# QualityMinds/cistgcn

Measured on AMD Instinct MI355X. Metric: sequences/sec (fwd+bwd) H3.6M 22-joint 50->25, higher is better.
Workload: dtype f32; 1 GPU; cistgcn64_b256_t50_v22; C=64, per_gpu_batch=256, global_batch=256, T_in=50, T_out=25, V=22, parallelism=dp1, graph=True, graph_branches=True, capture_kept=median, mixed_batches=False

## Files before the change

cistgcn_amd/_lib.py:

```python
import ctypes
import os
from ctypes import POINTER, c_double, c_float, c_int, c_int32, c_longlong, c_uint, c_ulonglong, c_void_p

HERE = os.path.dirname(os.path.abspath(__file__))
LIB_PATH = os.path.join(HERE, "libcistgcn_hip.so")

_handle = None
STAT_REPLICAS = 16
ALPHA_SLOTS = 64
_host_pointers_ok = False


class View4(ctypes.Structure):
    _fields_ = [("n", c_longlong * 4), ("s", c_longlong * 4)]


class NormAct(ctypes.Structure):
    _fields_ = [
        ("x", c_void_p), ("xv", View4),
        ("y", c_void_p), ("yv", View4),
        ("pre", c_void_p),
        ("add", c_void_p), ("av", View4),
        ("add_post", c_int),
        ("bn_mode", c_int),
# ... 209 lines not shown
    "cg_gate_head_scratch_floats": [c_int, c_int, c_int],
    "cg_context_heads_fwd": [POINTER(CtxHeads), P],
    "cg_context_heads_bwd": [POINTER(CtxHeads), P],
    "cg_context_heads_red_doubles": [c_int],
    "cg_map2adj_tail_fwd": [POINTER(AdjTail), c_int, c_int, P],
    "cg_map2adj_tail_bwd": [POINTER(AdjTail), c_int, c_int, P],
    "cg_map2adj_tail_ws_floats": [c_int],
    "cg_map2adj_tail_part_floats": [c_int, c_int, c_int],
    "cg_map2adj_tail_red_doubles": [c_int],
    "cg_augment_sequences": [P, P, P, P, P, P, P, P, P, P, c_int, c_int, c_int, c_int, P],
    "cg_map2adj_tail_geometry": [c_int, c_int, c_int, POINTER(c_int)],
    "cg_dstd_tail_geometry": [c_int, c_int, c_int, c_int, POINTER(c_int)],
    "cg_pointwise_maps_geometry": [c_int, c_int, c_int, c_int, POINTER(c_int), c_int, POINTER(c_int)],
    "cg_collapse_geometry": [c_int, c_int, c_int, c_int, c_int, c_int, POINTER(c_int)],
    "cg_fpn_conv_geometry": [c_int, c_int, c_int, c_int, c_int, POINTER(c_int)],
    "cg_stgcn_domain_geometry": [c_int, c_int, c_int, c_int, c_int, c_int, c_int, c_int, POINTER(c_int)],
    "cg_block_input_geometry": [c_int, c_int, c_int, c_int, POINTER(c_int)],
    "cg_norm_act_rows_per_block": [POINTER(View4)],
    "cg_glue_geometry": [c_int, c_int, c_int, POINTER(c_int)],
    "cg_mpjpe_sample_fwd": [P, P, P, c_int, c_int, P],
    "cg_mpjpe_sample_bwd": [P, P, P, P, c_int, c_int, P],
    "cg_attack_step": [POINTER(AttackStep), P],
    "cg_attack_step_max_floats": [],
    "cg_eval_metrics": [POINTER(EvalMetricsArgs), P],
    "cg_eval_metrics_ws_doubles": [c_int, c_int, c_int],
    "cg_attack_metrics": [POINTER(AttackMetricsArgs), P],
    "cg_attack_metrics_ws_doubles": [c_int, c_int, c_int],
    "cg_adam_flat": [P, P, P, P, LL, c_float, c_float, c_float, c_float, c_float, c_float, c_float, LL, P],
}
EXPORTS = tuple(sorted(_SIGNATURES))
# ... 33 lines not shown
```

cistgcn_amd/csrc/fpn_conv.hip:

```cpp
#include "cg_common.h"
#include "cg_phase.h"
#include "fpn_conv.h"

HIP_DYNAMIC_SHARED(unsigned char, cg_dyn_lds)

__device__ __forceinline__ void cg_fpn_store_quad(float* row, int p, int P, float a, float b, float c, float d) {
  if (p >= P) return;
  if ((P & 3) == 0) { *reinterpret_cast<float4*>(row + p) = make_float4(a, b, c, d); return; }
  *reinterpret_cast<float2*>(row + p) = make_float2(a, b);
  if (p + 2 < P) *reinterpret_cast<float2*>(row + p + 2) = make_float2(c, d);
}

#define CG_FPN_THREADS 512
#define CG_FPN_PAD 3

struct CgFpnGeom {
  int HP, WP, IMG;
  int P, PM;
  int K, KP, KS;
  int K2, KP2, KS2;
  int OM, CM;
  int per;
};
struct CgFpnArgs { CgFpnConv t; CgFpnGeom g; };

template <typename L, typename S>
__device__ __forceinline__ void cg_fpn_stage(int n, L load, S store) {
  for (int e0 = threadIdx.x; e0 < n; e0 += 8 * CG_FPN_THREADS) {
    float v[8];
#pragma unroll
    for (int j = 0; j < 8; ++j) { const int e = e0 + CG_FPN_THREADS * j; v[j] = e < n ? load(e) : 0.f; }
#pragma unroll
    for (int j = 0; j < 8; ++j) { const int e = e0 + CG_FPN_THREADS * j; if (e < n) store(e, v[j]); }
  }
}

__device__ __forceinline__ void cg_fpn_zero(float* img, int floats) {
  for (int e = threadIdx.x; e < floats / 4; e += CG_FPN_THREADS) reinterpret_cast<float4*>(img)[e] = make_float4(0.f, 0.f, 0.f, 0.f);
}
__device__ __forceinline__ void cg_fpn_fill(const float* __restrict__ src, long long sc, long long sh, int n, int H, int W, const CgFpnGeom& g, float* img) {
  const int P = H * W;
  cg_fpn_stage(n * P,
               [&](int e) { const int c = e / P, p = e - c * P, h = p / W; return src[c * sc + h * sh + (p - h * W)]; },
               [&](int e, float v) { const int c = e / P, p = e - c * P, h = p / W; img[c * g.IMG + (h + CG_FPN_PAD) * g.WP + (p - h * W) + CG_FPN_PAD] = v; });
}
__device__ __forceinline__ int cg_fpn_posoff(int p, int W, const CgFpnGeom& g) { const int h = p / W; return (h + CG_FPN_PAD) * g.WP + (p - h * W) + CG_FPN_PAD; }

__global__ __launch_bounds__(CG_FPN_THREADS) void cg_fpn_fwd_kernel(CgFpnArgs a) {
  const CgFpnConv& t = a.t; const CgFpnGeom& g = a.g;
  const int b = blockIdx.x, di = blockIdx.y, d = t.dil[di];
  float* sX = reinterpret_cast<float*>(cg_dyn_lds);
  float* sW = sX + t.C * g.IMG;
  int* sTap = reinterpret_cast<int*>(sW + g.OM * g.KS);
  int* sPos = sTap + g.KP;
  const int tid = threadIdx.x, lane = tid & 63, wave = __builtin_amdgcn_readfirstlane(tid >> 6), l15 = lane & 15, slot = lane >> 4;
  cg_fpn_zero(sX, t.C * g.IMG);
  cg_fpn_zero(sW, g.OM * g.KS);
  __syncthreads();
  cg_fpn_fill(t.x + (long long)b * t.xs[0], t.xs[1], t.xs[2], t.C, t.H, t.W, g, sX);
  cg_fpn_stage(t.O * g.K, [&](int e) { return t.w[di][e]; }, [&](int e, float v) { const int o = e / g.K; sW[o * g.KS + e - o * g.K] = v; });
  for (int k = tid; k < g.KP; k += CG_FPN_THREADS) {
    const int c = k / 9, ij = k - 9 * c, i = ij / 3, j = ij - 3 * i;
    sTap[k] = k < g.K ? c * g.IMG + d * (i - 1) * g.WP + d * (j - 1) : 0;
  }
  for (int p = tid; p < g.PM; p += CG_FPN_THREADS) sPos[p] = cg_fpn_posoff(p < g.P ? p : 0, t.W, g);
  __syncthreads();
  const int PT = g.PM / 16, OT = g.OM / 16, pairs = (PT + 1) / 2;
  float* yb = t.y[di] + (long long)b * t.O * g.P;
  for (int w = wave; w < pairs * OT; w += CG_FPN_THREADS / 64) {
    const int pr = w / OT, ot = w - pr * OT, pt0 = 2 * pr, pt1 = min(PT - 1, pt0 + 1);
    const int pa = sPos[16 * pt0 + l15], pb = sPos[16 * pt1 + l15];
    cg_f32x4 c0 = cg_f32x4{0.f, 0.f, 0.f, 0.f}, c1 = c0;
    const float* wp = sW + (16 * ot + l15) * g.KS + 4 * slot;
    for (int k0 = 0; k0 < g.KP; k0 += 16) {
      const float4 w4 = *reinterpret_cast<const float4*>(wp + k0);
      const int4 t4 = *reinterpret_cast<const int4*>(sTap + k0 + 4 * slot);
      const float wv[4] = {w4.x, w4.y, w4.z, w4.w};
      const int tv[4] = {t4.x, t4.y, t4.z, t4.w};
#pragma unroll
      for (int s = 0; s < 4; ++s) {
        c0 = __builtin_amdgcn_mfma_f32_16x16x4f32(sX[pa + tv[s]], wv[s], c0, 0, 0, 0);
        c1 = __builtin_amdgcn_mfma_f32_16x16x4f32(sX[pb + tv[s]], wv[s], c1, 0, 0, 0);
      }
    }
    const int o = 16 * ot + l15;
    if (o < t.O) {
      const float bias = t.bias[di] ? t.bias[di][o] : 0.f;
#pragma unroll
      for (int h = 0; h < 2; ++h) {
        if (h == 1 && pt1 == pt0) break;
        const int p = 16 * (h ? pt1 : pt0) + 4 * slot;
        const cg_f32x4 c = h ? c1 : c0;
        cg_fpn_store_quad(yb + (long long)o * g.P, p, g.P, c[0] + bias, c[1] + bias, c[2] + bias, c[3] + bias);
      }
    }
  }
}

#define CG_FPN_DXT 14

__global__ __launch_bounds__(CG_FPN_THREADS) void cg_fpn_dx_kernel(CgFpnArgs a) {
  const CgFpnConv& t = a.t; const CgFpnGeom& g = a.g;
  const int b = blockIdx.x;
  float* sD = reinterpret_cast<float*>(cg_dyn_lds);
  float* sW = sD + t.O * g.IMG;
  int* sTap = reinterpret_cast<int*>(sW + g.CM * g.KS2);
  int* sPos = sTap + g.KP2;
  const int tid = threadIdx.x, lane = tid & 63, wave = __builtin_amdgcn_readfirstlane(tid >> 6), l15 = lane & 15, slot = lane >> 4, nw = CG_FPN_THREADS / 64;
  const int PT = g.PM / 16, CT = g.CM / 16;
  cg_f32x4 acc[CG_FPN_DXT];
#pragma unroll
  for (int u = 0; u < CG_FPN_DXT; ++u) acc[u] = cg_f32x4{0.f, 0.f, 0.f, 0.f};
  for (int p = tid; p < g.PM; p += CG_FPN_THREADS) sPos[p] = cg_fpn_posoff(p < g.P ? p : 0, t.W, g);
  cg_fpn_zero(sD, t.O * g.IMG);
  cg_fpn_zero(sW, g.CM * g.KS2);
  for (int di = 0; di < t.n; ++di) {
    const int d = t.dil[di];
    __syncthreads();
    cg_fpn_fill(t.dy[di] + (long long)b * t.O * g.P, g.P, t.W, t.O, t.H, t.W, g, sD);
    cg_fpn_stage(t.O * t.C * 9, [&](int e) { return t.w[di][e]; },
                 [&](int e, float v) { const int oc = e / 9, ij = e - 9 * oc, o = oc / t.C, c = oc - o * t.C; sW[c * g.KS2 + o * 9 + ij] = v; });
    for (int k = tid; k < g.KP2; k += CG_FPN_THREADS) {
      const int o = k / 9, ij = k - 9 * o, i = ij / 3, j = ij - 3 * i;
      sTap[k] = k < g.K2 ? o * g.IMG - d * (i - 1) * g.WP - d * (j - 1) : 0;
    }
    __syncthreads();
#pragma unroll
    for (int u = 0; u < CG_FPN_DXT; u += 2) {
      const int id0 = u * nw + wave, id1 = (u + 1) * nw + wave;
      if (id0 < PT * CT) {
        const bool two = id1 < PT * CT;
        const int pt0 = id0 / CT, ct0 = id0 - pt0 * CT, pt1 = two ? id1 / CT : pt0, ct1 = two ? id1 - pt1 * CT : ct0;
        const int pa = sPos[16 * pt0 + l15], pb = sPos[16 * pt1 + l15];
        const float* wp0 = sW + (16 * ct0 + l15) * g.KS2 + 4 * slot;
        const float* wp1 = sW + (16 * ct1 + l15) * g.KS2 + 4 * slot;
        cg_f32x4 c0 = acc[u], c1 = acc[u + 1];
#pragma unroll 3
        for (int k0 = 0; k0 < g.KP2; k0 += 16) {
          const float4 w0 = *reinterpret_cast<const float4*>(wp0 + k0), w1 = *reinterpret_cast<const float4*>(wp1 + k0);
          const int4 t4 = *reinterpret_cast<const int4*>(sTap + k0 + 4 * slot);
          const float a0[4] = {sD[pa + t4.x], sD[pa + t4.y], sD[pa + t4.z], sD[pa + t4.w]};
          const float a1[4] = {sD[pb + t4.x], sD[pb + t4.y], sD[pb + t4.z], sD[pb + t4.w]};
          const float v0[4] = {w0.x, w0.y, w0.z, w0.w}, v1[4] = {w1.x, w1.y, w1.z, w1.w};
#pragma unroll
          for (int s4 = 0; s4 < 4; ++s4) {
            c0 = __builtin_amdgcn_mfma_f32_16x16x4f32(a0[s4], v0[s4], c0, 0, 0, 0);
            c1 = __builtin_amdgcn_mfma_f32_16x16x4f32(a1[s4], v1[s4], c1, 0, 0, 0);
          }
        }
        acc[u] = c0;
        if (two) acc[u + 1] = c1;
      }
    }
  }
  float* dxb = t.dx + (long long)b * t.C * g.P;
#pragma unroll
  for (int u = 0; u < CG_FPN_DXT; ++u) {
    const int id = u * nw + wave;
    if (id < PT * CT) {
      const int pt = id / CT, ct = id - pt * CT, c = 16 * ct + l15, p = 16 * pt + 4 * slot;
      if (c < t.C) cg_fpn_store_quad(dxb + (long long)c * g.P, p, g.P, acc[u][0], acc[u][1], acc[u][2], acc[u][3]);
    }
  }
}

#define CG_FPN_DWT 16

__global__ __launch_bounds__(CG_FPN_THREADS) void cg_fpn_dw_kernel(CgFpnArgs a) {
  const CgFpnConv& t = a.t; const CgFpnGeom& g = a.g;
  const int di = blockIdx.y, d = t.dil[di];
  const int b0 = blockIdx.x * g.per, b1 = min(t.B, b0 + g.per);
  if (b0 >= t.B) return;
  const int DS = g.PM + 4;
  float* sX = reinterpret_cast<float*>(cg_dyn_lds);
  float* sD = sX + t.C * g.IMG;
  int* sTap = reinterpret_cast<int*>(sD + g.OM * DS);
  int* sPos = sTap + g.KP;
  const int tid = threadIdx.x, lane = tid & 63, wave = __builtin_amdgcn_readfirstlane(tid >> 6), l15 = lane & 15, slot = lane >> 4, nw = CG_FPN_THREADS / 64;
  const int OT = g.OM / 16, KT = g.KP / 16;
  cg_f32x4 acc[CG_FPN_DWT];
#pragma unroll
  for (int u = 0; u < CG_FPN_DWT; ++u) acc[u] = cg_f32x4{0.f, 0.f, 0.f, 0.f};
  float bsum = 0.f, bsum1 = 0.f;
  for (int k = tid; k < g.KP; k += CG_FPN_THREADS) {
    const int c = k / 9, ij = k - 9 * c, i = ij / 3, j = ij - 3 * i;
    sTap[k] = k < g.K ? c * g.IMG + d * (i - 1) * g.WP + d * (j - 1) : 0;
  }
  for (int p = tid; p < g.PM; p += CG_FPN_THREADS) sPos[p] = cg_fpn_posoff(p < g.P ? p : 0, t.W, g);
  for (int e = tid; e < g.OM * DS; e += CG_FPN_THREADS) sD[e] = 0.f;
  cg_fpn_zero(sX, t.C * g.IMG);
  for (int b = b0; b < b1; ++b) {
    __syncthreads();
    cg_fpn_fill(t.x + (long long)b * t.xs[0], t.xs[1], t.xs[2], t.C, t.H, t.W, g, sX);
    const float* dyb = t.dy[di] + (long long)b * t.O * g.P;
    if ((g.P & 3) == 0) {
#pragma unroll 4
      for (int e = tid; e < t.O * (g.P / 4); e += CG_FPN_THREADS) {
        const int o = e / (g.P / 4), p = 4 * (e - o * (g.P / 4));
        *reinterpret_cast<float4*>(sD + o * DS + p) = *reinterpret_cast<const float4*>(dyb + (long long)o * g.P + p);
      }
    } else {
#pragma unroll 4
      for (int e = tid; e < t.O * (g.P / 2); e += CG_FPN_THREADS) {
        const int o = e / (g.P / 2), p = 2 * (e - o * (g.P / 2));
        *reinterpret_cast<float2*>(sD + o * DS + p) = *reinterpret_cast<const float2*>(dyb + (long long)o * g.P + p);
      }
    }
    __syncthreads();
#pragma unroll
    for (int u = 0; u < CG_FPN_DWT; u += 2) {
      const int id0 = u * nw + wave, id1 = (u + 1) * nw + wave;
      if (id0 < OT * KT) {
        const bool two = id1 < OT * KT;
        const int ot0 = id0 / KT, kt0 = id0 - ot0 * KT, ot1 = two ? id1 / KT : ot0, kt1 = two ? id1 - ot1 * KT : kt0;
        const int tap0 = sTap[16 * kt0 + l15], tap1 = sTap[16 * kt1 + l15];
        const float* dp0 = sD + (16 * ot0 + l15) * DS + 4 * slot;
        const float* dp1 = sD + (16 * ot1 + l15) * DS + 4 * slot;
        cg_f32x4 c0 = acc[u], c1 = acc[u + 1];
        float bs0 = 0.f, bs1 = 0.f;
#pragma unroll 2
        for (int p0 = 0; p0 < g.PM; p0 += 16) {
          const float4 d0 = *reinterpret_cast<const float4*>(dp0 + p0), d1 = *reinterpret_cast<const float4*>(dp1 + p0);
          const int4 q4 = *reinterpret_cast<const int4*>(sPos + p0 + 4 * slot);
          const float x0[4] = {sX[tap0 + q4.x], sX[tap0 + q4.y], sX[tap0 + q4.z], sX[tap0 + q4.w]};
          const float x1[4] = {sX[tap1 + q4.x], sX[tap1 + q4.y], sX[tap1 + q4.z], sX[tap1 + q4.w]};
          const float e0[4] = {d0.x, d0.y, d0.z, d0.w}, e1[4] = {d1.x, d1.y, d1.z, d1.w};
          bs0 += (d0.x + d0.y) + (d0.z + d0.w); bs1 += (d1.x + d1.y) + (d1.z + d1.w);
#pragma unroll
          for (int s4 = 0; s4 < 4; ++s4) {
            c0 = __builtin_amdgcn_mfma_f32_16x16x4f32(e0[s4], x0[s4], c0, 0, 0, 0);
            c1 = __builtin_amdgcn_mfma_f32_16x16x4f32(e1[s4], x1[s4], c1, 0, 0, 0);
          }
        }
        acc[u] = c0;
        if (two) acc[u + 1] = c1;
        if (kt0 == 0) { if (ot0) bsum1 += bs0; else bsum += bs0; }
        if (two && kt1 == 0) { if (ot1) bsum1 += bs1; else bsum += bs1; }
      }
    }
  }
  float* ws = t.ws + ((long long)blockIdx.x * t.n + di) * (t.O * g.K + t.O);
#pragma unroll
  for (int u = 0; u < CG_FPN_DWT; ++u) {
    const int id = u * nw + wave;
    if (id < OT * KT) {
      const int ot = id / KT, kt = id - ot * KT, k = 16 * kt + l15;
#pragma unroll
      for (int q = 0; q < 4; ++q) {
        const int o = 16 * ot + 4 * slot + q;
        if (o < t.O && k < g.K) ws[o * g.K + k] = acc[u][q];
      }
    }
  }
  bsum += __shfl_xor(bsum, 16, 64); bsum += __shfl_xor(bsum, 32, 64);
  bsum1 += __shfl_xor(bsum1, 16, 64); bsum1 += __shfl_xor(bsum1, 32, 64);
  float* sB = reinterpret_cast<float*>(cg_dyn_lds);
  __syncthreads();
  if (slot == 0) { sB[wave * 16 + l15] = bsum; sB[(nw + wave) * 16 + l15] = bsum1; }
  __syncthreads();
  if (tid < 32 && tid < t.O) {
    float s0 = 0.f;
// ... 6 lines not shown
  __shared__ float red[4][64];
  const CgFpnConv& t = a.t; const CgFpnGeom& g = a.g;
  const int di = blockIdx.y, n = t.O * g.K + t.O, e = blockIdx.x * 64 + (threadIdx.x & 63), part = threadIdx.x >> 6;
  float s = 0.f;
  if (e < n)
    for (int w = part; w < nwg; w += 4) s += t.ws[((long long)w * t.n + di) * n + e];
  red[part][threadIdx.x & 63] = s;
  __syncthreads();
  if (part == 0 && e < n) {
    s = (red[0][threadIdx.x] + red[1][threadIdx.x]) + (red[2][threadIdx.x] + red[3][threadIdx.x]);
    if (e < t.O * g.K) { if (t.dw[di]) t.dw[di][e] = s; }
    else if (t.db[di]) t.db[di][e - t.O * g.K] = s;
  }
}

static int cg_fpn_geometry(const CgFpnConv* t, CgFpnGeom* g) {
  if (!t || t->n <= 0 || t->n > 3) return CG_EARG;
  if (t->B <= 0 || t->C <= 0 || t->C > 64 || t->O <= 0 || t->O > 32 || t->H <= 0 || t->W <= 0) return CG_ESHAPE;
  for (int i = 0; i < t->n; ++i) if (t->dil[i] < 1 || t->dil[i] > CG_FPN_PAD) return CG_ESHAPE;
  g->HP = t->H + 2 * CG_FPN_PAD; g->WP = t->W + 2 * CG_FPN_PAD; g->IMG = g->HP * g->WP;
  g->P = t->H * t->W; g->PM = (g->P + 15) & ~15;
  if ((g->P & 1) || g->PM > 256) return CG_ESHAPE;
  g->K = t->C * 9; g->KP = (g->K + 15) & ~15; g->KS = g->KP + 4;
  g->K2 = t->O * 9; g->KP2 = (g->K2 + 15) & ~15; g->KS2 = g->KP2 + 4;
  g->OM = (t->O + 15) & ~15; g->CM = (t->C + 15) & ~15;
  const int nwg = t->B < 170 ? t->B : 170;
  g->per = (t->B + nwg - 1) / nwg;
  if ((g->PM / 16) * (g->CM / 16) > CG_FPN_DXT * 4) return CG_ESHAPE;
  if ((g->OM / 16) * (g->KP / 16) > CG_FPN_DWT * 4) return CG_ESHAPE;
  return CG_OK;
}
static size_t cg_fpn_lds_fwd(const CgFpnConv* t, const CgFpnGeom& g) { return ((size_t)t->C * g.IMG + (size_t)g.OM * g.KS + g.KP + g.PM) * 4; }
static size_t cg_fpn_lds_dx(const CgFpnConv* t, const CgFpnGeom& g) { return ((size_t)t->O * g.IMG + (size_t)g.CM * g.KS2 + g.KP2 + g.PM) * 4; }
static size_t cg_fpn_lds_dw(const CgFpnConv* t, const CgFpnGeom& g) { return ((size_t)t->C * g.IMG + (size_t)g.OM * (g.PM + 4) + g.KP + g.PM) * 4; }

static int cg_fpn_dw_nwg(int B, const CgFpnGeom& g) { return (B + g.per - 1) / g.per; }
extern "C" int cg_fpn_conv_geometry(int B, int C, int O, int H, int W, int* out) {
  if (!out) return CG_EARG;
  CgFpnConv t = {};
  t.B = B; t.C = C; t.O = O; t.H = H; t.W = W; t.n = 1; t.dil[0] = 1;
  CgFpnGeom g;
  const int st = cg_fpn_geometry(&t, &g);
  if (st != CG_OK) return st;
  out[0] = g.per; out[1] = cg_fpn_dw_nwg(B, g);
  return CG_OK;
}

extern "C" int cg_fpn_conv_supported(int B, int C, int O, int H, int W) {
  CgFpnConv t = {};
  t.B = B; t.C = C; t.O = O; t.H = H; t.W = W; t.n = 1; t.dil[0] = 1;
  CgFpnGeom g;
  if (cg_fpn_geometry(&t, &g) != CG_OK) return 0;
  const size_t cap = 160 * 1024;
  return cg_fpn_lds_fwd(&t, g) <= cap && cg_fpn_lds_dx(&t, g) <= cap && cg_fpn_lds_dw(&t, g) <= cap;
}
extern "C" long long cg_fpn_conv_ws_floats(int B, int C, int O, int n) { return (long long)(B < 170 ? B : 170) * n * (O * C * 9 + O); }

extern "C" int cg_fpn_conv_fwd(const CgFpnConv* t, void* stream_) {
  CgFpnArgs a;
  int st = cg_fpn_geometry(t, &a.g);
  if (st != CG_OK) return st;
  a.t = *t;
  if (!t->x) return CG_EARG;
  for (int i = 0; i < t->n; ++i) if (!t->w[i] || !t->y[i]) return CG_EARG;
  const size_t lds = cg_fpn_lds_fwd(t, a.g);
  if (lds > 160 * 1024) return CG_ESHAPE;
  hipError_t e = cg_lds_limit((const void*)cg_fpn_fwd_kernel, lds);
  if (e != hipSuccess) return (int)e;
  hipLaunchKernelGGL(cg_fpn_fwd_kernel, dim3((unsigned)t->B, (unsigned)t->n), dim3(CG_FPN_THREADS), lds, (hipStream_t)stream_, a);
  return cg_launch_status();
}

extern "C" int cg_fpn_conv_bwd(const CgFpnConv* t, void* stream_) {
  CgFpnArgs a;
  int st = cg_fpn_geometry(t, &a.g);
  if (st != CG_OK) return st;
  a.t = *t;
  if (!t->x || !t->ws) return CG_EARG;
  for (int i = 0; i < t->n; ++i) if (!t->w[i] || !t->dy[i]) return CG_EARG;
  hipStream_t stream = (hipStream_t)stream_;
  if (t->dx) {
    const size_t lds = cg_fpn_lds_dx(t, a.g);
    if (lds > 160 * 1024) return CG_ESHAPE;
    hipError_t e = cg_lds_limit((const void*)cg_fpn_dx_kernel, lds);
    if (e != hipSuccess) return (int)e;
    hipLaunchKernelGGL(cg_fpn_dx_kernel, dim3((unsigned)t->B), dim3(CG_FPN_THREADS), lds, stream, a);
    st = cg_launch_status();
    if (st != CG_OK) return st;
  }
  const size_t lds = cg_fpn_lds_dw(t, a.g);
  if (lds > 160 * 1024) return CG_ESHAPE;
  hipError_t e = cg_lds_limit((const void*)cg_fpn_dw_kernel, lds);
  if (e != hipSuccess) return (int)e;
  const int nwg = cg_fpn_dw_nwg(t->B, a.g);
  hipLaunchKernelGGL(cg_fpn_dw_kernel, dim3((unsigned)nwg, (unsigned)t->n), dim3(CG_FPN_THREADS), lds, stream, a);
  st = cg_launch_status();
  if (st != CG_OK) return st;
  const int nel = t->O * a.g.K + t->O;
  hipLaunchKernelGGL(cg_fpn_fold_kernel, dim3((unsigned)((nel + 63) / 64), (unsigned)t->n), dim3(256), 0, stream, a, nwg);
  return cg_launch_status();
}
```

include/cistgcn_hip.h:

```cpp
#ifndef CISTGCN_HIP_H
#define CISTGCN_HIP_H
#include <stdint.h>
#ifdef __cplusplus
extern "C" {
#endif

#define CG_STAT_REPLICAS 16
#define CG_ALPHA_SLOTS 64

typedef struct CgView4 {
  long long n[4];
  long long s[4];
} CgView4;

int cg_contract(const float* A, const float* X, float* Y, const float* bias, double* stats, const int32_t* tables,
                int G, int M, int N, int K, int splitk, int a_kfast, int x_kfast,
                long long y_dense_numel, void* stream);

typedef struct CgContractDesc {
  const float* A; const float* X; float* Y; const float* bias; double* stats; const int32_t* tab;
  int G, M, N, K, splitk, kchunk , a_kfast, x_kfast;
  int accumulate;
  int x_vec;
  int stat_ch;
// ... 242 lines not shown
  float* tap[2];
  const float* dy[2];
  double* red;
  float* dx;
  float* dw[2]; float* dgamma[2]; float* dbeta[2]; float* dalpha[2];
} CgCtxHeads;
int cg_context_heads_fwd(const CgCtxHeads* t, void* stream);
int cg_context_heads_bwd(const CgCtxHeads* t, void* stream);
long long cg_context_heads_red_doubles(int C);

int cg_map2adj_tail_geometry(int B, int Kc, int J, int* out);
int cg_dstd_tail_geometry(int B, int C, int T, int V, int* out);
int cg_pointwise_maps_geometry(int B, int Cin, int P, int n, const int* M, int bwd, int* out);
int cg_collapse_geometry(int B, int C, int T, int V, int O, int cols, int* out);
int cg_fpn_conv_geometry(int B, int C, int O, int H, int W, int* out);
int cg_stgcn_domain_geometry(int B, int Cin, int Cout, int T, int V, int domain, int bwd, int kind, int* out);
int cg_block_input_geometry(int B, int C, int T, int V, int* out);
int cg_norm_act_rows_per_block(const CgView4* xv);
int cg_glue_geometry(int C, int T, int V, int* out);

int cg_gather_joints(const float* x, float* y, const int32_t* idx, long long rows, int Jin, int Jout, void* stream);
int cg_eval_scatter_mpjpe(const float* pred, const float* target, float* out, float* frame_err, const int32_t* src,
                          int B, int To, int J32, int J22, void* stream);

int cg_augment_sequences(const float* raw, const float* params, float* sample, float* target, float* target_vel,
                         float* target_gvel, float* processed, float* sample_vel, const float* noise_tab, const int32_t* perm,
                         int B, int L, int J, int input_n, void* stream);

int cg_adam_flat(float* param, const float* grad, float* exp_avg, float* exp_avg_sq, long long n, float lr, float beta1,
                 float beta2, float eps, float weight_decay, float grad_scale, float clip_value, long long step_count,
// ... 41 lines not shown
```

Measured before the change: 14760 sequences/sec.

## Stream batches through persistent FPN conv workgroups with register prefetch and resident weights

The FPN dilated conv forward and dx kernels change from one workgroup per sample (and per dilation) to a capped grid of persistent workgroups that each loop over several samples. All dilation weights stay resident in LDS when they fit, and the next sample's image or weights are prefetched into registers while MFMA tiles run, with double-buffered operand reads in the inner loop. The goal is to hide global-load latency and cut per-workgroup setup and weight restaging. The cost is more register pressure and less parallelism per workgroup; a new geometry query is exported.

Measured after the change: 14830 sequences/sec, median of 6. No clear change (+0.4%).

```diff
diff --git a/cistgcn_amd/_lib.py b/cistgcn_amd/_lib.py
--- a/cistgcn_amd/_lib.py
+++ b/cistgcn_amd/_lib.py
@@ -247,6 +247,7 @@
     "cg_pointwise_maps_geometry": [c_int, c_int, c_int, c_int, POINTER(c_int), c_int, POINTER(c_int)],
     "cg_collapse_geometry": [c_int, c_int, c_int, c_int, c_int, c_int, POINTER(c_int)],
     "cg_fpn_conv_geometry": [c_int, c_int, c_int, c_int, c_int, POINTER(c_int)],
+    "cg_fpn_conv_stream_geometry": [c_int, c_int, c_int, c_int, c_int, c_int, POINTER(c_int)],
     "cg_stgcn_domain_geometry": [c_int, c_int, c_int, c_int, c_int, c_int, c_int, c_int, POINTER(c_int)],
     "cg_block_input_geometry": [c_int, c_int, c_int, c_int, POINTER(c_int)],
     "cg_norm_act_rows_per_block": [POINTER(View4)],
diff --git a/cistgcn_amd/csrc/fpn_conv.hip b/cistgcn_amd/csrc/fpn_conv.hip
--- a/cistgcn_amd/csrc/fpn_conv.hip
+++ b/cistgcn_amd/csrc/fpn_conv.hip
@@ -13,6 +13,9 @@
 
 #define CG_FPN_THREADS 512
 #define CG_FPN_PAD 3
+#define CG_FPN_PF 32
+#define CG_FPN_LDS (160 * 1024)
+#define CG_FPN_MAX_WG 256
 
 struct CgFpnGeom {
   int HP, WP, IMG;
@@ -21,9 +24,14 @@
   int K2, KP2, KS2;
   int OM, CM;
   int per;
+  int fper, fnwg, fres;
+  int xper, xnwg, xres;
 };
 struct CgFpnArgs { CgFpnConv t; CgFpnGeom g; };
 
+__device__ __forceinline__ void cg_fpn_zero(float* img, int floats) {
+  for (int e = threadIdx.x; e < floats / 4; e += CG_FPN_THREADS) reinterpret_cast<float4*>(img)[e] = make_float4(0.f, 0.f, 0.f, 0.f);
+}
 template <typename L, typename S>
 __device__ __forceinline__ void cg_fpn_stage(int n, L load, S store) {
   for (int e0 = threadIdx.x; e0 < n; e0 += 8 * CG_FPN_THREADS) {
@@ -33,10 +41,6 @@
 #pragma unroll
     for (int j = 0; j < 8; ++j) { const int e = e0 + CG_FPN_THREADS * j; if (e < n) store(e, v[j]); }
   }
-}
-
-__device__ __forceinline__ void cg_fpn_zero(float* img, int floats) {
-  for (int e = threadIdx.x; e < floats / 4; e += CG_FPN_THREADS) reinterpret_cast<float4*>(img)[e] = make_float4(0.f, 0.f, 0.f, 0.f);
 }
 __device__ __forceinline__ void cg_fpn_fill(const float* __restrict__ src, long long sc, long long sh, int n, int H, int W, const CgFpnGeom& g, float* img) {
   const int P = H * W;
@@ -46,125 +50,270 @@
 }
 __device__ __forceinline__ int cg_fpn_posoff(int p, int W, const CgFpnGeom& g) { const int h = p / W; return (h + CG_FPN_PAD) * g.WP + (p - h * W) + CG_FPN_PAD; }
 
+struct CgFpnWalk { int q, r, dq, dr, len; };
+__device__ __forceinline__ CgFpnWalk cg_fpn_walk(int len) {
+  CgFpnWalk w;
+  w.len = len; w.q = (int)threadIdx.x / len; w.r = (int)threadIdx.x - w.q * len; w.dq = CG_FPN_THREADS / len; w.dr = CG_FPN_THREADS - w.dq * len;
+  return w;
+}
+__device__ __forceinline__ void cg_fpn_step(CgFpnWalk& w) { w.q += w.dq; w.r += w.dr; if (w.r >= w.len) { w.r -= w.len; ++w.q; } }
+__device__ __forceinline__ int cg_fpn_row(int p, float rW) { return (int)(((float)p + 0.5f) * rW); }
+
+__device__ __forceinline__ void cg_fpn_img_request(const float* __restrict__ src, long long sc, long long sh, int rows, int W, float rW, CgFpnWalk w, float (&v)[CG_FPN_PF]) {
+  CG_OPAQUE_V(w.q); CG_OPAQUE_V(w.r);
+#pragma unroll
+  for (int j = 0; j < CG_FPN_PF; ++j) {
+    if ((j & 7) == 0 && j * CG_FPN_THREADS >= rows * w.len) break;
+    const int h = cg_fpn_row(w.r, rW);
+    v[j] = w.q < rows ? src[w.q * sc + h * sh + (w.r - h * W)] : 0.f;
+    cg_fpn_step(w);
+  }
+}
+__device__ __forceinline__ void cg_fpn_img_commit(float* img, int rows, int W, float rW, const CgFpnGeom& g, CgFpnWalk w, const float (&v)[CG_FPN_PF]) {
+  CG_OPAQUE_V(w.q); CG_OPAQUE_V(w.r);
+#pragma unroll
+  for (int j = 0; j < CG_FPN_PF; ++j) {
+    if ((j & 7) == 0 && j * CG_FPN_THREADS >= rows * w.len) break;
+    const int h = cg_fpn_row(w.r, rW);
+    if (w.q < rows) img[w.q * g.IMG + (h + CG_FPN_PAD) * g.WP + (w.r - h * W) + CG_FPN_PAD] = v[j];
+    cg_fpn_step(w);
+  }
+}
+__device__ __forceinline__ void cg_fpn_w_request(const float* __restrict__ wd, int n, float (&v)[CG_FPN_PF]) {
+  int tid = threadIdx.x;
+  CG_OPAQUE_V(tid);
+#pragma unroll
+  for (int j = 0; j < CG_FPN_PF; ++j) {
+    if ((j & 7) == 0 && j * CG_FPN_THREADS >= n) break;
+    const int e = j * CG_FPN_THREADS + tid;
+    v[j] = e < n ? wd[e] : 0.f;
+  }
+}
+template <bool TR>
+__device__ __forceinline__ void cg_fpn_w_commit(float* sW, int O, int stride, CgFpnWalk w, const float (&v)[CG_FPN_PF]) {
+  CG_OPAQUE_V(w.q); CG_OPAQUE_V(w.r);
+#pragma unroll
+  for (int j = 0; j < CG_FPN_PF; ++j) {
+    if ((j & 7) == 0 && j * CG_FPN_THREADS >= O * w.len) break;
+    if (w.q < O) {
+      if (TR) { const int c = w.r / 9; sW[c * stride + w.q * 9 + (w.r - 9 * c)] = v[j]; }
+      else sW[w.q * stride + w.r] = v[j];
+    }
+    cg_fpn_step(w);
+  }
+}
+__device__ __forceinline__ void cg_fpn_taps(int* sTap, int K, int KP, int d, int sign, const CgFpnGeom& g) {
+  for (int k = threadIdx.x; k < KP; k += CG_FPN_THREADS) {
+    const int c = k / 9, ij = k - 9 * c, i = ij / 3, j = ij - 3 * i;
+    sTap[k] = k < K ? c * g.IMG + sign * (d * (i - 1) * g.WP + d * (j - 1)) : 0;
+  }
+}
+
+struct CgFpnOps { float xa[4], xb[4], v0[4], v1[4]; };
+__device__ __forceinline__ void cg_fpn_ops_read(CgFpnOps& o, const float* sImg, const float* w, int wstep, int pa, int pb, const int4& t4) {
+  const float4 w0 = *reinterpret_cast<const float4*>(w), w1 = *reinterpret_cast<const float4*>(w + wstep);
+  o.xa[0] = sImg[pa + t4.x]; o.xa[1] = sImg[pa + t4.y]; o.xa[2] = sImg[pa + t4.z]; o.xa[3] = sImg[pa + t4.w];
+  o.xb[0] = sImg[pb + t4.x]; o.xb[1] = sImg[pb + t4.y]; o.xb[2] = sImg[pb + t4.z]; o.xb[3] = sImg[pb + t4.w];
+  o.v0[0] = w0.x; o.v0[1] = w0.y; o.v0[2] = w0.z; o.v0[3] = w0.w;
+  o.v1[0] = w1.x; o.v1[1] = w1.y; o.v1[2] = w1.z; o.v1[3] = w1.w;
+}
+template <bool TWO>
+__device__ __forceinline__ void cg_fpn_tiles(const float* sImg, const float* wrow, int wstep, const int* tap, int pa, int pb, int KP, cg_f32x4 (&c)[4]) {
+  CgFpnOps cur, nxt;
+  int4 t4 = *reinterpret_cast<const int4*>(tap);
+  cg_fpn_ops_read(cur, sImg, wrow, wstep, pa, pb, t4);
+  t4 = *reinterpret_cast<const int4*>(tap + min(16, KP - 16));
+  for (int k0 = 0; k0 < KP; k0 += 16) {
+    const int k1 = min(k0 + 16, KP - 16), k2 = min(k0 + 32, KP - 16);
+    cg_fpn_ops_read(nxt, sImg, wrow + k1, wstep, pa, pb, t4);
+    t4 = *reinterpret_cast<const int4*>(tap + k2);
+    __builtin_amdgcn_sched_barrier(0);
+#pragma unroll
+    for (int s = 0; s < 4; ++s) {
+      c[0] = __builtin_amdgcn_mfma_f32_16x16x4f32(cur.xa[s], cur.v0[s], c[0], 0, 0, 0);
+      c[1] = __builtin_amdgcn_mfma_f32_16x16x4f32(cur.xb[s], cur.v0[s], c[1], 0, 0, 0);
+      if (TWO) {
+        c[2] = __builtin_amdgcn_mfma_f32_16x16x4f32(cur.xa[s], cur.v1[s], c[2], 0, 0, 0);
+        c[3] = __builtin_amdgcn_mfma_f32_16x16x4f32(cur.xb[s], cur.v1[s], c[3], 0, 0, 0);
+      }
+    }
+    __builtin_amdgcn_sched_barrier(0);
+    cur = nxt;
+  }
+}
+
+template <bool TWO>
+__device__ __forceinline__ void cg_fpn_fwd_task(const CgFpnConv& t, const CgFpnGeom& g, const float* sX, const float* sWd, const int* sTapd, const int* sPos,
+                                                int b, int di, int pr, int l15, int slot) {
+  const int PT = g.PM / 16, pt0 = 2 * pr, pt1 = min(PT - 1, pt0 + 1);
+  cg_f32x4 c[4];
+#pragma unroll
+  for (int u = 0; u < 4; ++u) c[u] = cg_f32x4{0.f, 0.f, 0.f, 0.f};
+  cg_fpn_tiles<TWO>(sX, sWd + l15 * g.KS + 4 * slot, TWO ? 16 * g.KS : 0, sTapd + 4 * slot, sPos[16 * pt0 + l15], sPos[16 * pt1 + l15], g.KP, c);
+  float* yb = t.y[di] + (long long)b * t.O * g.P;
+#pragma unroll
+  for (int u = 0; u < (TWO ? 4 : 2); ++u) {
+    const int o = 16 * (u >> 1) + l15, pt = (u & 1) ? pt1 : pt0;
+    if ((u & 1) && pt1 == pt0) continue;
+    if (o < t.O) {
+      const float bias = t.bias[di] ? t.bias[di][o] : 0.f;
+      cg_fpn_store_quad(yb + (long long)o * g.P, 16 * pt + 4 * slot, g.P, c[u][0] + bias, c[u][1] + bias, c[u][2] + bias, c[u][3] + bias);
+    }
+  }
+}
+
 __global__ __launch_bounds__(CG_FPN_THREADS) void cg_fpn_fwd_kernel(CgFpnArgs a) {
   const CgFpnConv& t = a.t; const CgFpnGeom& g = a.g;
-  const int b = blockIdx.x, di = blockIdx.y, d = t.dil[di];
+  const int b0 = blockIdx.x * g.fper, b1 = min(t.B, b0 + g.fper), nres = g.fres ? t.n : 1;
+  if (b0 >= t.B) return;
   float* sX = reinterpret_cast<float*>(cg_dyn_lds);
   float* sW = sX + t.C * g.IMG;
-  int* sTap = reinterpret_cast<int*>(sW + g.OM * g.KS);
-  int* sPos = sTap + g.KP;
-  const int tid = threadIdx.x, lane = tid & 63, wave = __builtin_amdgcn_readfirstlane(tid >> 6), l15 = lane & 15, slot = lane >> 4;
+  int* sTap = reinterpret_cast<int*>(sW + nres * g.OM * g.KS);
+  int* sPos = sTap + nres * g.KP;
+  const int tid = threadIdx.x, lane = tid & 63, wave = __builtin_amdgcn_readfirstlane(tid >> 6), l15 = lane & 15, slot = lane >> 4, nw = CG_FPN_THREADS / 64;
+  const float rW = 1.f / (float)t.W;
+  const CgFpnWalk wx = cg_fpn_walk(g.P), ww = cg_fpn_walk(g.K);
+  const int WM = g.OM * g.KS, TPD = (g.PM / 16 + 1) / 2;
+  float pf[CG_FPN_PF], pw[CG_FPN_PF];
   cg_fpn_zero(sX, t.C * g.IMG);
-  cg_fpn_zero(sW, g.OM * g.KS);
-  __syncthreads();
-  cg_fpn_fill(t.x + (long long)b * t.xs[0], t.xs[1], t.xs[2], t.C, t.H, t.W, g, sX);
-  cg_fpn_stage(t.O * g.K, [&](int e) { return t.w[di][e]; }, [&](int e, float v) { const int o = e / g.K; sW[o * g.KS + e - o * g.K] = v; });
-  for (int k = tid; k < g.KP; k += CG_FPN_THREADS) {
-    const int c = k / 9, ij = k - 9 * c, i = ij / 3, j = ij - 3 * i;
-    sTap[k] = k < g.K ? c * g.IMG + d * (i - 1) * g.WP + d * (j - 1) : 0;
-  }
+  cg_fpn_zero(sW, nres * WM);
   for (int p = tid; p < g.PM; p += CG_FPN_THREADS) sPos[p] = cg_fpn_posoff(p < g.P ? p : 0, t.W, g);
   __syncthreads();
-  const int PT = g.PM / 16, OT = g.OM / 16, pairs = (PT + 1) / 2;
-  float* yb = t.y[di] + (long long)b * t.O * g.P;
-  for (int w = wave; w < pairs * OT; w += CG_FPN_THREADS / 64) {
-    const int pr = w / OT, ot = w - pr * OT, pt0 = 2 * pr, pt1 = min(PT - 1, pt0 + 1);
-    const int pa = sPos[16 * pt0 + l15], pb = sPos[16 * pt1 + l15];
-    cg_f32x4 c0 = cg_f32x4{0.f, 0.f, 0.f, 0.f}, c1 = c0;
-    const float* wp = sW + (16 * ot + l15) * g.KS + 4 * slot;
-    for (int k0 = 0; k0 < g.KP; k0 += 16) {
-      const float4 w4 = *reinterpret_cast<const float4*>(wp + k0);
-      const int4 t4 = *reinterpret_cast<const int4*>(sTap + k0 + 4 * slot);
-      const float wv[4] = {w4.x, w4.y, w4.z, w4.w};
-      const int tv[4] = {t4.x, t4.y, t4.z, t4.w};
-#pragma unroll
-      for (int s = 0; s < 4; ++s) {
-        c0 = __builtin_amdgcn_mfma_f32_16x16x4f32(sX[pa + tv[s]], wv[s], c0, 0, 0, 0);
-        c1 = __builtin_amdgcn_mfma_f32_16x16x4f32(sX[pb + tv[s]], wv[s], c1, 0, 0, 0);
-      }
-    }
-    const int o = 16 * ot + l15;
-    if (o < t.O) {
-      const float bias = t.bias[di] ? t.bias[di][o] : 0.f;
-#pragma unroll
-      for (int h = 0; h < 2; ++h) {
-        if (h == 1 && pt1 == pt0) break;
-        const int p = 16 * (h ? pt1 : pt0) + 4 * slot;
-        const cg_f32x4 c = h ? c1 : c0;
-        cg_fpn_store_quad(yb + (long long)o * g.P, p, g.P, c[0] + bias, c[1] + bias, c[2] + bias, c[3] + bias);
-      }
-    }
-  }
-}
-
-#define CG_FPN_DXT 14
+  cg_fpn_img_request(t.x + (long long)b0 * t.xs[0], t.xs[1], t.xs[2], t.C, t.W, rW, wx, pf);
+  for (int r = 0; r < nres; ++r) {
+    cg_fpn_w_request(t.w[r], t.O * g.K, pw);
+    cg_fpn_taps(sTap + r * g.KP, g.K, g.KP, t.dil[r], 1, g);
+    cg_fpn_w_commit<false>(sW + r * WM, t.O, g.KS, ww, pw);
+  }
+  cg_fpn_img_commit(sX, t.C, t.W, rW, g, wx, pf);
+  __syncthreads();
+  const int nph = g.fres ? 1 : t.n, dpp = g.fres ? t.n : 1;
+  for (int b = b0; b < b1; ++b) {
+    const bool more = b + 1 < b1;
+    for (int ph = 0; ph < nph; ++ph) {
+      const bool last = ph == nph - 1;
+      const int nx = last ? 0 : ph + 1;
+      const bool nwt = nph > 1 && (!last || more), nim = more && last;
+      if (nwt) cg_fpn_w_request(t.w[nx], t.O * g.K, pw);
+      if (nim) cg_fpn_img_request(t.x + (long long)(b + 1) * t.xs[0], t.xs[1], t.xs[2], t.C, t.W, rW, wx, pf);
+      for (int w = wave; w < dpp * TPD; w += nw) {
+        const int dl = w / TPD, pr = w - dl * TPD;
+        if (g.OM == 32) cg_fpn_fwd_task<true>(t, g, sX, sW + dl * WM, sTap + dl * g.KP, sPos, b, ph + dl, pr, l15, slot);
+        else cg_fpn_fwd_task<false>(t, g, sX, sW + dl * WM, sTap + dl * g.KP, sPos, b, ph + dl, pr, l15, slot);
+      }
+      if (nwt || nim) {
+        __syncthreads();
+        if (nwt) { cg_fpn_w_commit<false>(sW, t.O, g.KS, ww, pw); cg_fpn_taps(sTap, g.K, g.KP, t.dil[nx], 1, g); }
+        if (nim) cg_fpn_img_commit(sX, t.C, t.W, rW, g, wx, pf);
+        __syncthreads();
+      }
+    }
+  }
+}
+
+#define CG_FPN_DXR 2
 
 __global__ __launch_bounds__(CG_FPN_THREADS) void cg_fpn_dx_kernel(CgFpnArgs a) {
   const CgFpnConv& t = a.t; const CgFpnGeom& g = a.g;
-  const int b = blockIdx.x;
+  const int b0 = blockIdx.x * g.xper, b1 = min(t.B, b0 + g.xper), nres = g.xres ? t.n : 1;
+  if (b0 >= t.B) return;
   float* sD = reinterpret_cast<float*>(cg_dyn_lds);
   float* sW = sD + t.O * g.IMG;
-  int* sTap = reinterpret_cast<int*>(sW + g.CM * g.KS2);
-  int* sPos = sTap + g.KP2;
+  int* sTap = reinterpret_cast<int*>(sW + nres * g.CM * g.KS2);
+  int* sPos = sTap + nres * g.KP2;
   const int tid = threadIdx.x, lane = tid & 63, wave = __builtin_amdgcn_readfirstlane(tid >> 6), l15 = lane & 15, slot = lane >> 4, nw = CG_FPN_THREADS / 64;
-  const int PT = g.PM / 16, CT = g.CM / 16;
-  cg_f32x4 acc[CG_FPN_DXT];
-#pragma unroll
-  for (int u = 0; u < CG_FPN_DXT; ++u) acc[u] = cg_f32x4{0.f, 0.f, 0.f, 0.f};
+  const float rW = 1.f / (float)t.W;
+  const CgFpnWalk wd = cg_fpn_walk(g.P), ww = cg_fpn_walk(g.K);
+  const int WM = g.CM * g.KS2, PT = g.PM / 16, CT = g.CM / 16, CP = (CT + 1) / 2, NT = ((PT + 1) / 2) * CP;
+  const long long ds = (long long)t.O * g.P;
+  float pf[CG_FPN_PF], pw[CG_FPN_PF];
+  cg_fpn_zero(sD, t.O * g.IMG);
+  cg_fpn_zero(sW, nres * WM);
   for (int p = tid; p < g.PM; p += CG_FPN_THREADS) sPos[p] = cg_fpn_posoff(p < g.P ? p : 0, t.W, g);
-  cg_fpn_zero(sD, t.O * g.IMG);
-  cg_fpn_zero(sW, g.CM * g.KS2);
-  for (int di = 0; di < t.n; ++di) {
-    const int d = t.dil[di];
-    __syncthreads();
-    cg_fpn_fill(t.dy[di] + (long long)b * t.O * g.P, g.P, t.W, t.O, t.H, t.W, g, sD);
-    cg_fpn_stage(t.O * t.C * 9, [&](int e) { return t.w[di][e]; },
-                 [&](int e, float v) { const int oc = e / 9, ij = e - 9 * oc, o = oc / t.C, c = oc - o * t.C; sW[c * g.KS2 + o * 9 + ij] = v; });
-    for (int k = tid; k < g.KP2; k += CG_FPN_THREADS) {
-      const int o = k / 9, ij = k - 9 * o, i = ij / 3, j = ij - 3 * i;
-      sTap[k] = k < g.K2 ? o * g.IMG - d * (i - 1) * g.WP - d * (j - 1) : 0;
-    }
-    __syncthreads();
-#pragma unroll
-    for (int u = 0; u < CG_FPN_DXT; u += 2) {
-      const int id0 = u * nw + wave, id1 = (u + 1) * nw + wave;
-      if (id0 < PT * CT) {
-        const bool two = id1 < PT * CT;
-        const int pt0 = id0 / CT, ct0 = id0 - pt0 * CT, pt1 = two ? id1 / CT : pt0, ct1 = two ? id1 - pt1 * CT : ct0;
-        const int pa = sPos[16 * pt0 + l15], pb = sPos[16 * pt1 + l15];
-        const float* wp0 = sW + (16 * ct0 + l15) * g.KS2 + 4 * slot;
-        const float* wp1 = sW + (16 * ct1 + l15) * g.KS2 + 4 * slot;
-        cg_f32x4 c0 = acc[u], c1 = acc[u + 1];
-#pragma unroll 3
-        for (int k0 = 0; k0 < g.KP2; k0 += 16) {
-          const float4 w0 = *reinterpret_cast<const float4*>(wp0 + k0), w1 = *reinterpret_cast<const float4*>(wp1 + k0);
-          const int4 t4 = *reinterpret_cast<const int4*>(sTap + k0 + 4 * slot);
-          const float a0[4] = {sD[pa + t4.x], sD[pa + t4.y], sD[pa + t4.z], sD[pa + t4.w]};
-          const float a1[4] = {sD[pb + t4.x], sD[pb + t4.y], sD[pb + t4.z], sD[pb + t4.w]};
-          const float v0[4] = {w0.x, w0.y, w0.z, w0.w}, v1[4] = {w1.x, w1.y, w1.z, w1.w};
-#pragma unroll
-          for (int s4 = 0; s4 < 4; ++s4) {
-            c0 = __builtin_amdgcn_mfma_f32_16x16x4f32(a0[s4], v0[s4], c0, 0, 0, 0);
-            c1 = __builtin_amdgcn_mfma_f32_16x16x4f32(a1[s4], v1[s4], c1, 0, 0, 0);
-          }
+  __syncthreads();
+  cg_fpn_img_request(t.dy[0] + b0 * ds, g.P, t.W, t.O, t.W, rW, wd, pf);
+  for (int r = 0; r < nres; ++r) {
+    cg_fpn_w_request(t.w[r], t.O * g.K, pw);
+    cg_fpn_taps(sTap + r * g.KP2, g.K2, g.KP2, t.dil[r], -1, g);
+    cg_fpn_w_commit<true>(sW + r * WM, t.O, g.KS2, ww, pw);
+  }
+  cg_fpn_img_commit(sD, t.O, t.W, rW, g, wd, pf);
+  __syncthreads();
+  for (int b = b0; b < b1; ++b) {
+    cg_f32x4 acc[CG_FPN_DXR][4];
+#pragma unroll
+    for (int r = 0; r < CG_FPN_DXR; ++r)
+#pragma unroll
+      for (int u = 0; u < 4; ++u) acc[r][u] = cg_f32x4{0.f, 0.f, 0.f, 0.f};
+    for (int di = 0; di < t.n; ++di) {
+      const int nd = di + 1 < t.n ? di + 1 : 0, nb = di + 1 < t.n ? b : b + 1;
+      const bool nim = nb < b1, nwt = nim && !g.xres && t.n > 1;
+      if (nim) cg_fpn_img_request(t.dy[nd] + nb * ds, g.P, t.W, t.O, t.W, rW, wd, pf);
+      if (nwt) cg_fpn_w_request(t.w[nd], t.O * g.K, pw);
+      const float* sWd = sW + (g.xres ? di * WM : 0);
+      const int* sTapd = sTap + (g.xres ? di * g.KP2 : 0);
+#pragma unroll
+      for (int r = 0; r < CG_FPN_DXR; ++r) {
+        const int q = r * nw + wave;
+        if (q < NT) {
+          const int pr = q / CP, ct0 = 2 * (q - pr * CP), pt0 = 2 * pr, pt1 = min(PT - 1, pt0 + 1);
+          const float* wrow = sWd + (16 * ct0 + l15) * g.KS2 + 4 * slot;
+          const int pa = sPos[16 * pt0 + l15], pb = sPos[16 * pt1 + l15];
+          if (CT > 1) cg_fpn_tiles<true>(sD, wrow, ct0 + 1 < CT ? 16 * g.KS2 : 0, sTapd + 4 * slot, pa, pb, g.KP2, acc[r]);
+          else cg_fpn_tiles<false>(sD, wrow, 0, sTapd + 4 * slot, pa, pb, g.KP2, acc[r]);
         }
-        acc[u] = c0;
-        if (two) acc[u + 1] = c1;
-      }
-    }
-  }
-  float* dxb = t.dx + (long long)b * t.C * g.P;
-#pragma unroll
-  for (int u = 0; u < CG_FPN_DXT; ++u) {
-    const int id = u * nw + wave;
-    if (id < PT * CT) {
-      const int pt = id / CT, ct = id - pt * CT, c = 16 * ct + l15, p = 16 * pt + 4 * slot;
-      if (c < t.C) cg_fpn_store_quad(dxb + (long long)c * g.P, p, g.P, acc[u][0], acc[u][1], acc[u][2], acc[u][3]);
+      }
+      if (nim) {
+        __syncthreads();
+        cg_fpn_img_commit(sD, t.O, t.W, rW, g, wd, pf);
+        if (nwt) { cg_fpn_w_commit<true>(sW, t.O, g.KS2, ww, pw); cg_fpn_taps(sTap, g.K2, g.KP2, t.dil[nd], -1, g); }
+        __syncthreads();
+      }
+    }
+    float* dxb = t.dx + (long long)b * t.C * g.P;
+#pragma unroll
+    for (int r = 0; r < CG_FPN_DXR; ++r) {
+      const int q = r * nw + wave;
+      if (q < NT) {
+        const int pr = q / CP, ct0 = 2 * (q - pr * CP), pt0 = 2 * pr;
+#pragma unroll
+        for (int u = 0; u < 4; ++u) {
+          const int pt = pt0 + (u & 1), ct = ct0 + (u >> 1), c = 16 * ct + l15;
+          if (pt < PT && ct < CT && c < t.C) cg_fpn_store_quad(dxb + (long long)c * g.P, 16 * pt + 4 * slot, g.P, acc[r][u][0], acc[r][u][1], acc[r][u][2], acc[r][u][3]);
+        }
+      }
     }
   }
 }
 
 #define CG_FPN_DWT 16
+
+template <bool SHAREX>
+__device__ __forceinline__ void cg_fpn_dw_tiles(const float* sX, const float* dp0, const float* dp1, const int* pos, int tap0, int tap1, int PM,
+                                                cg_f32x4& c0, cg_f32x4& c1, float& bs0, float& bs1) {
+  for (int p0 = 0; p0 < PM; p0 += 16) {
+    const float4 d0 = *reinterpret_cast<const float4*>(dp0 + p0);
+    const float4 d1 = SHAREX ? *reinterpret_cast<const float4*>(dp1 + p0) : d0;
+    const int4 q4 = *reinterpret_cast<const int4*>(pos + p0);
+    const float x0[4] = {sX[tap0 + q4.x], sX[tap0 + q4.y], sX[tap0 + q4.z], sX[tap0 + q4.w]};
+    float x1[4] = {x0[0], x0[1], x0[2], x0[3]};
+    if (!SHAREX) { x1[0] = sX[tap1 + q4.x]; x1[1] = sX[tap1 + q4.y]; x1[2] = sX[tap1 + q4.z]; x1[3] = sX[tap1 + q4.w]; }
+    const float e0[4] = {d0.x, d0.y, d0.z, d0.w}, e1[4] = {d1.x, d1.y, d1.z, d1.w};
+    bs0 += (d0.x + d0.y) + (d0.z + d0.w); bs1 += (d1.x + d1.y) + (d1.z + d1.w);
+#pragma unroll
+    for (int s4 = 0; s4 < 4; ++s4) {
+      c0 = __builtin_amdgcn_mfma_f32_16x16x4f32(e0[s4], x0[s4], c0, 0, 0, 0);
+      c1 = __builtin_amdgcn_mfma_f32_16x16x4f32(e1[s4], x1[s4], c1, 0, 0, 0);
+    }
+  }
+}
+__device__ __forceinline__ bool cg_fpn_dw_tile(int u, int wave, int OT, int KT, int& ot, int& kt) {
+  const int nw = CG_FPN_THREADS / 64;
+  if (OT == 2) { ot = u & 1; kt = (u >> 1) * nw + wave; return kt < KT; }
+  const int id = u * nw + wave;
+  ot = id / KT; kt = id - ot * KT;
+  return id < OT * KT;
+}
 
 __global__ __launch_bounds__(CG_FPN_THREADS) void cg_fpn_dw_kernel(CgFpnArgs a) {
   const CgFpnConv& t = a.t; const CgFpnGeom& g = a.g;
@@ -182,10 +331,7 @@
 #pragma unroll
   for (int u = 0; u < CG_FPN_DWT; ++u) acc[u] = cg_f32x4{0.f, 0.f, 0.f, 0.f};
   float bsum = 0.f, bsum1 = 0.f;
-  for (int k = tid; k < g.KP; k += CG_FPN_THREADS) {
-    const int c = k / 9, ij = k - 9 * c, i = ij / 3, j = ij - 3 * i;
-    sTap[k] = k < g.K ? c * g.IMG + d * (i - 1) * g.WP + d * (j - 1) : 0;
-  }
+  cg_fpn_taps(sTap, g.K, g.KP, d, 1, g);
   for (int p = tid; p < g.PM; p += CG_FPN_THREADS) sPos[p] = cg_fpn_posoff(p < g.P ? p : 0, t.W, g);
   for (int e = tid; e < g.OM * DS; e += CG_FPN_THREADS) sD[e] = 0.f;
   cg_fpn_zero(sX, t.C * g.IMG);
@@ -209,29 +355,17 @@
     __syncthreads();
 #pragma unroll
     for (int u = 0; u < CG_FPN_DWT; u += 2) {
-      const int id0 = u * nw + wave, id1 = (u + 1) * nw + wave;
-      if (id0 < OT * KT) {
-        const bool two = id1 < OT * KT;
-        const int ot0 = id0 / KT, kt0 = id0 - ot0 * KT, ot1 = two ? id1 / KT : ot0, kt1 = two ? id1 - ot1 * KT : kt0;
+      int ot0, kt0, ot1, kt1;
+      if (cg_fpn_dw_tile(u, wave, OT, KT, ot0, kt0)) {
+        const bool two = cg_fpn_dw_tile(u + 1, wave, OT, KT, ot1, kt1);
+        if (!two) { ot1 = ot0; kt1 = kt0; }
         const int tap0 = sTap[16 * kt0 + l15], tap1 = sTap[16 * kt1 + l15];
         const float* dp0 = sD + (16 * ot0 + l15) * DS + 4 * slot;
         const float* dp1 = sD + (16 * ot1 + l15) * DS + 4 * slot;
         cg_f32x4 c0 = acc[u], c1 = acc[u + 1];
         float bs0 = 0.f, bs1 = 0.f;
-#pragma unroll 2
-        for (int p0 = 0; p0 < g.PM; p0 += 16) {
-          const float4 d0 = *reinterpret_cast<const float4*>(dp0 + p0), d1 = *reinterpret_cast<const float4*>(dp1 + p0);
-          const int4 q4 = *reinterpret_cast<const int4*>(sPos + p0 + 4 * slot);
-          const float x0[4] = {sX[tap0 + q4.x], sX[tap0 + q4.y], sX[tap0 + q4.z], sX[tap0 + q4.w]};
-          const float x1[4] = {sX[tap1 + q4.x], sX[tap1 + q4.y], sX[tap1 + q4.z], sX[tap1 + q4.w]};
-          const float e0[4] = {d0.x, d0.y, d0.z, d0.w}, e1[4] = {d1.x, d1.y, d1.z, d1.w};
-          bs0 += (d0.x + d0.y) + (d0.z + d0.w); bs1 += (d1.x + d1.y) + (d1.z + d1.w);
-#pragma unroll
-          for (int s4 = 0; s4 < 4; ++s4) {
-            c0 = __builtin_amdgcn_mfma_f32_16x16x4f32(e0[s4], x0[s4], c0, 0, 0, 0);
-            c1 = __builtin_amdgcn_mfma_f32_16x16x4f32(e1[s4], x1[s4], c1, 0, 0, 0);
-          }
-        }
+        if (OT == 2) cg_fpn_dw_tiles<true>(sX, dp0, dp1, sPos + 4 * slot, tap0, tap1, g.PM, c0, c1, bs0, bs1);
+        else cg_fpn_dw_tiles<false>(sX, dp0, dp1, sPos + 4 * slot, tap0, tap1, g.PM, c0, c1, bs0, bs1);
         acc[u] = c0;
         if (two) acc[u + 1] = c1;
         if (kt0 == 0) { if (ot0) bsum1 += bs0; else bsum += bs0; }
@@ -242,9 +376,9 @@
   float* ws = t.ws + ((long long)blockIdx.x * t.n + di) * (t.O * g.K + t.O);
 #pragma unroll
   for (int u = 0; u < CG_FPN_DWT; ++u) {
-    const int id = u * nw + wave;
-    if (id < OT * KT) {
-      const int ot = id / KT, kt = id - ot * KT, k = 16 * kt + l15;
+    int ot, kt;
+    if (cg_fpn_dw_tile(u, wave, OT, KT, ot, kt)) {
+      const int k = 16 * kt + l15;
 #pragma unroll
       for (int q = 0; q < 4; ++q) {
         const int o = 16 * ot + 4 * slot + q;
@@ -281,11 +415,16 @@
   }
 }
 
+static size_t cg_fpn_lds_fwd(const CgFpnConv* t, const CgFpnGeom& g, int nres) { return ((size_t)t->C * g.IMG + (size_t)nres * (g.OM * g.KS + g.KP) + g.PM) * 4; }
+static size_t cg_fpn_lds_dx(const CgFpnConv* t, const CgFpnGeom& g, int nres) { return ((size_t)t->O * g.IMG + (size_t)nres * (g.CM * g.KS2 + g.KP2) + g.PM) * 4; }
+static size_t cg_fpn_lds_dw(const CgFpnConv* t, const CgFpnGeom& g) { return ((size_t)t->C * g.IMG + (size_t)g.OM * (g.PM + 4) + g.KP + g.PM) * 4; }
+
 static int cg_fpn_geometry(const CgFpnConv* t, CgFpnGeom* g) {
   if (!t || t->n <= 0 || t->n > 3) return CG_EARG;
   if (t->B <= 0 || t->C <= 0 || t->C > 64 || t->O <= 0 || t->O > 32 || t->H <= 0 || t->W <= 0) return CG_ESHAPE;
   for (int i = 0; i < t->n; ++i) if (t->dil[i] < 1 || t->dil[i] > CG_FPN_PAD) return CG_ESHAPE;
-  g->HP = t->H + 2 * CG_FPN_PAD; g->WP = t->W + 2 * CG_FPN_PAD; g->IMG = g->HP * g->WP;
+  g->HP = t->H + 2 * CG_FPN_PAD; g->WP = t->W + 2 * CG_FPN_PAD;
+  g->IMG = (g->HP * g->WP + 3) & ~3;
   g->P = t->H * t->W; g->PM = (g->P + 15) & ~15;
   if ((g->P & 1) || g->PM > 256) return CG_ESHAPE;
   g->K = t->C * 9; g->KP = (g->K + 15) & ~15; g->KS = g->KP + 4;
@@ -293,13 +432,15 @@
   g->OM = (t->O + 15) & ~15; g->CM = (t->C + 15) & ~15;
   const int nwg = t->B < 170 ? t->B : 170;
   g->per = (t->B + nwg - 1) / nwg;
-  if ((g->PM / 16) * (g->CM / 16) > CG_FPN_DXT * 4) return CG_ESHAPE;
+  if ((g->PM / 16) * (g->CM / 16) > 56) return CG_ESHAPE;
   if ((g->OM / 16) * (g->KP / 16) > CG_FPN_DWT * 4) return CG_ESHAPE;
+  if (t->C * g->P > CG_FPN_PF * CG_FPN_THREADS || t->O * g->P > CG_FPN_PF * CG_FPN_THREADS || t->O * g->K > CG_FPN_PF * CG_FPN_THREADS) return CG_ESHAPE;
+  g->fper = g->xper = (t->B + CG_FPN_MAX_WG - 1) / CG_FPN_MAX_WG;
+  g->fnwg = g->xnwg = (t->B + g->fper - 1) / g->fper;
+  g->fres = cg_fpn_lds_fwd(t, *g, t->n) <= CG_FPN_LDS;
+  g->xres = cg_fpn_lds_dx(t, *g, t->n) <= CG_FPN_LDS;
   return CG_OK;
 }
-static size_t cg_fpn_lds_fwd(const CgFpnConv* t, const CgFpnGeom& g) { return ((size_t)t->C * g.IMG + (size_t)g.OM * g.KS + g.KP + g.PM) * 4; }
-static size_t cg_fpn_lds_dx(const CgFpnConv* t, const CgFpnGeom& g) { return ((size_t)t->O * g.IMG + (size_t)g.CM * g.KS2 + g.KP2 + g.PM) * 4; }
-static size_t cg_fpn_lds_dw(const CgFpnConv* t, const CgFpnGeom& g) { return ((size_t)t->C * g.IMG + (size_t)g.OM * (g.PM + 4) + g.KP + g.PM) * 4; }
 
 static int cg_fpn_dw_nwg(int B, const CgFpnGeom& g) { return (B + g.per - 1) / g.per; }
 extern "C" int cg_fpn_conv_geometry(int B, int C, int O, int H, int W, int* out) {
@@ -312,14 +453,26 @@
   out[0] = g.per; out[1] = cg_fpn_dw_nwg(B, g);
   return CG_OK;
 }
+extern "C" int cg_fpn_conv_stream_geometry(int B, int C, int O, int H, int W, int n, int* out) {
+  if (!out || n < 1 || n > 3) return CG_EARG;
+  CgFpnConv t = {};
+  t.B = B; t.C = C; t.O = O; t.H = H; t.W = W; t.n = n;
+  for (int i = 0; i < n; ++i) t.dil[i] = i + 1;
+  CgFpnGeom g;
+  const int st = cg_fpn_geometry(&t, &g);
+  if (st != CG_OK) return st;
+  out[0] = g.fper; out[1] = g.fnwg; out[2] = g.fres;
+  out[3] = g.xper; out[4] = g.xnwg; out[5] = g.xres;
+  return CG_OK;
+}
 
 extern "C" int cg_fpn_conv_supported(int B, int C, int O, int H, int W) {
   CgFpnConv t = {};
   t.B = B; t.C = C; t.O = O; t.H = H; t.W = W; t.n = 1; t.dil[0] = 1;
   CgFpnGeom g;
   if (cg_fpn_geometry(&t, &g) != CG_OK) return 0;
-  const size_t cap = 160 * 1024;
-  return cg_fpn_lds_fwd(&t, g) <= cap && cg_fpn_lds_dx(&t, g) <= cap && cg_fpn_lds_dw(&t, g) <= cap;
+  const size_t cap = CG_FPN_LDS;
+  return cg_fpn_lds_fwd(&t, g, 1) <= cap && cg_fpn_lds_dx(&t, g, 1) <= cap && cg_fpn_lds_dw(&t, g) <= cap;
 }
 extern "C" long long cg_fpn_conv_ws_floats(int B, int C, int O, int n) { return (long long)(B < 170 ? B : 170) * n * (O * C * 9 + O); }
 
@@ -330,11 +483,11 @@
   a.t = *t;
   if (!t->x) return CG_EARG;
   for (int i = 0; i < t->n; ++i) if (!t->w[i] || !t->y[i]) return CG_EARG;
-  const size_t lds = cg_fpn_lds_fwd(t, a.g);
-  if (lds > 160 * 1024) return CG_ESHAPE;
+  const size_t lds = cg_fpn_lds_fwd(t, a.g, a.g.fres ? t->n : 1);
+  if (lds > CG_FPN_LDS) return CG_ESHAPE;
   hipError_t e = cg_lds_limit((const void*)cg_fpn_fwd_kernel, lds);
   if (e != hipSuccess) return (int)e;
-  hipLaunchKernelGGL(cg_fpn_fwd_kernel, dim3((unsigned)t->B, (unsigned)t->n), dim3(CG_FPN_THREADS), lds, (hipStream_t)stream_, a);
+  hipLaunchKernelGGL(cg_fpn_fwd_kernel, dim3((unsigned)a.g.fnwg), dim3(CG_FPN_THREADS), lds, (hipStream_t)stream_, a);
   return cg_launch_status();
 }
 
@@ -347,16 +500,16 @@
   for (int i = 0; i < t->n; ++i) if (!t->w[i] || !t->dy[i]) return CG_EARG;
   hipStream_t stream = (hipStream_t)stream_;
   if (t->dx) {
-    const size_t lds = cg_fpn_lds_dx(t, a.g);
-    if (lds > 160 * 1024) return CG_ESHAPE;
+    const size_t lds = cg_fpn_lds_dx(t, a.g, a.g.xres ? t->n : 1);
+    if (lds > CG_FPN_LDS) return CG_ESHAPE;
     hipError_t e = cg_lds_limit((const void*)cg_fpn_dx_kernel, lds);
     if (e != hipSuccess) return (int)e;
-    hipLaunchKernelGGL(cg_fpn_dx_kernel, dim3((unsigned)t->B), dim3(CG_FPN_THREADS), lds, stream, a);
+    hipLaunchKernelGGL(cg_fpn_dx_kernel, dim3((unsigned)a.g.xnwg), dim3(CG_FPN_THREADS), lds, stream, a);
     st = cg_launch_status();
     if (st != CG_OK) return st;
   }
   const size_t lds = cg_fpn_lds_dw(t, a.g);
-  if (lds > 160 * 1024) return CG_ESHAPE;
+  if (lds > CG_FPN_LDS) return CG_ESHAPE;
   hipError_t e = cg_lds_limit((const void*)cg_fpn_dw_kernel, lds);
   if (e != hipSuccess) return (int)e;
   const int nwg = cg_fpn_dw_nwg(t->B, a.g);
diff --git a/include/cistgcn_hip.h b/include/cistgcn_hip.h
--- a/include/cistgcn_hip.h
+++ b/include/cistgcn_hip.h
@@ -280,6 +280,7 @@
 int cg_pointwise_maps_geometry(int B, int Cin, int P, int n, const int* M, int bwd, int* out);
 int cg_collapse_geometry(int B, int C, int T, int V, int O, int cols, int* out);
 int cg_fpn_conv_geometry(int B, int C, int O, int H, int W, int* out);
+int cg_fpn_conv_stream_geometry(int B, int C, int O, int H, int W, int n, int* out);
 int cg_stgcn_domain_geometry(int B, int Cin, int Cout, int T, int V, int domain, int bwd, int kind, int* out);
 int cg_block_input_geometry(int B, int C, int T, int V, int* out);
 int cg_norm_act_rows_per_block(const CgView4* xv);
```
